# kehlert/ellp

Hardware: AMD Instinct MI355X
Metric: simplex pivots/sec (dense LP, primal, tableau resident in HBM) (higher is better)
Workload: dtype f64

## Files before the change

### ellp_amd/csrc/engine/ellp_engine.hip

```cpp
#include <hip/hip_runtime.h>
#include <dlfcn.h>
#include <rccl/rccl.h>

#include <algorithm>
#include <chrono>
#include <cmath>
#include <cstdarg>
#include <cstdint>
#include <cstdio>
#include <cstdlib>
#include <cstring>
#include <limits>
#include <memory>
#include <mutex>
#include <optional>
#include <vector>

#include "ellp_hip.h"
#include "ellp_lu_dev.h"

namespace {

constexpr int ST_RUNNING = 100;
constexpr int ST_NEED_MAINT = 101;
// ... 3064 lines not shown
void launch_dual_close(ellp_engine *e);
void maintain_inverse(ellp_engine *e, bool reactive = false, bool rebuild = false) {
    launch_dual_close(e);
    if (e->lagged) hipLaunchKernelGGL(k_drop_open, dim3(1), dim3(1), 0, e->stream, e->st);
    e->lag_open = false;
    if (rebuild) launch_refactor(e);
    else launch_refresh(e);
    const char *mode = getenv("ELLP_RESYNC");
    const bool want = mode && mode[0] == '0' ? false : (mode && mode[0] == '1' ? reactive : true);
    if (want) launch_resync(e, 0);
}

void reconcile_counters(ellp_engine *e) {
    const uint64_t ran = e->h_st->iters >= e->iters_seen ? e->h_st->iters - e->iters_seen : 0;
    const uint64_t lost = e->enqueued > ran ? e->enqueued - ran : 0;
    if (lost) {
        e->since_refactor = e->since_refactor > lost ? e->since_refactor - lost : 0;
        e->since_btran = e->since_btran > lost ? e->since_btran - lost : 0;
        e->since_drift = e->since_drift > lost ? e->since_drift - lost : 0;
    }
    e->enqueued = 0;
    e->iters_seen = e->h_st->iters;
}

void adopt_fin(ellp_engine *e) {
    if (e->h_st->status != ST_RUNNING || !e->h_st->fin) return;
    static int32_t fin_status;
    fin_status = e->h_st->fin - 1;
    (void)hipMemcpyAsync(&e->st->status, &fin_status, sizeof(int32_t), hipMemcpyHostToDevice, e->stream);
    (void)hipStreamSynchronize(e->stream);
    e->h_st->status = fin_status;
}

bool service_maintenance_request(ellp_engine *e) {
    if (e->h_st->status != ST_NEED_MAINT && !(e->h_st->status == ST_RUNNING && e->h_st->tiny)) return false;
    const int32_t running = ST_RUNNING, zero = 0;
    const bool rebuild = e->h_st->need_rebuild != 0;
    (void)hipMemcpyAsync(&e->st->status, &running, sizeof(int32_t), hipMemcpyHostToDevice, e->stream);
    (void)hipMemcpyAsync(&e->st->tiny, &zero, sizeof(int32_t), hipMemcpyHostToDevice, e->stream);
    (void)hipMemcpyAsync(&e->st->need_rebuild, &zero, sizeof(int32_t), hipMemcpyHostToDevice, e->stream);
    e->h_st->status = ST_RUNNING;
    e->h_st->tiny = 0;
    e->h_st->need_rebuild = 0;
    maintain_inverse(e, true, rebuild);
    e->maint_chain = 1;
    (void)hipStreamSynchronize(e->stream);
    e->maint_requests += 1;
    return true;
}

void launch_drift_check(ellp_engine *e) {
    if (e->drift_every <= 0) return;
    if (++e->since_drift < (uint64_t)e->drift_every) return;
    e->since_drift = 0;
    e->drift_checks += 1;
    DriftArgs a{e->A_B, e->A_N, e->d, e->colshard ? e->aq_cur : nullptr, e->upart, e->st, e->m, e->ld, e->btran_rows, e->btran_tiles, e->drift_tol};
    const int64_t half = e->ld >> 1;
    hipLaunchKernelGGL(k_drift_part, dim3((unsigned)((half + 255) / 256), (unsigned)e->btran_tiles), dim3(256), 0,
                       e->stream, a);
    hipLaunchKernelGGL(k_drift_reduce, dim3((unsigned)((e->m + WAVE - 1) / WAVE)), dim3(WAVE), 0, e->stream, a);
}

void launch_price2(ellp_engine *e, int use_pend) {
    Price2Args a{};
    a.p.A_N = e->A_N; a.p.W0 = e->W; a.p.W1 = e->W2; a.p.u = nullptr; a.p.c_N = e->c_N; a.p.Nb = e->Nb;
    a.p.N_index = e->N_index; a.p.dd = nullptr; a.p.xc = Xchg{e->X, e->seg, e->nbs, e->cpb}; a.p.st = e->st;
    a.p.ld = e->ld; a.p.nN = e->nN; a.p.cpb = e->cpb; a.p.block0 = e->rank * e->nbs; a.p.eps = e->eps;
    a.p.vs_row = e->vs_row; a.p.vs_val = e->vs_val; a.pos_hint = e->pos_hint;
    a.u0 = e->u; a.u1 = e->u + e->ld; a.W0 = e->W; a.W1 = e->W2;
    a.d = e->d; a.lam = e->lam; a.bmin = e->bmin; a.bsec = e->bmin + e->m; a.bidx = e->bidx; a.binfo = e->binfo; a.dpos = e->dpos;
    a.A_N = e->A_N; a.A_B = e->A_B; a.aq_save = e->aq_save; a.c_B = e->c_B; a.c_N = e->c_N; a.x = e->x;
    a.lb = e->lb; a.ub = e->ub; a.kind = e->kindv; a.B_index = e->B_index; a.N_index = e->N_index; a.Nb = e->Nb;
    a.m = e->m; a.rpb = e->upd2_rows; a.use_pend = use_pend; a.ill_tol = e->ill_tol;
    a.guard_abs = (e->cert_large && !e->guard_off) ? e->guard_abs : 0.0;
    a.aq_cur = e->colshard ? e->aq_cur : nullptr; a.own0 = e->own0; a.own1 = e->own1;
    a.trace = Trace{e->trace_obj, e->trace_it, e->trace_len};
    int mine = e->nblocks - a.p.block0;
    if (mine > e->nbs) mine = e->nbs;
    if (mine < 0) mine = 0;
    const dim3 g(mine + P2_BOOK), b(256);
    const size_t lds = e->price2_lds;
    if (e->colshard) {
        if (e->price_wave) {
            hipLaunchKernelGGL((k_price2_wave<true>), g, b, lds + sizeof(double) * (size_t)e->ld, e->stream, a);
            return;
        }
        if (e->price_nt) {
            switch (e->priceT) {
            case 1: hipLaunchKernelGGL((k_price2<1, true, true>), g, b, lds, e->stream, a); break;
            case 2: hipLaunchKernelGGL((k_price2<2, true, true>), g, b, lds, e->stream, a); break;
            case 4: hipLaunchKernelGGL((k_price2<4, true, true>), g, b, lds, e->stream, a); break;
            case 8: hipLaunchKernelGGL((k_price2<8, true, true>), g, b, lds, e->stream, a); break;
            default: hipLaunchKernelGGL((k_price2<16, true, true>), g, b, lds, e->stream, a); break;
            }
        } else {
            switch (e->priceT) {
            case 1: hipLaunchKernelGGL((k_price2<1, false, true>), g, b, lds, e->stream, a); break;
            case 2: hipLaunchKernelGGL((k_price2<2, false, true>), g, b, lds, e->stream, a); break;
            case 4: hipLaunchKernelGGL((k_price2<4, false, true>), g, b, lds, e->stream, a); break;
            case 8: hipLaunchKernelGGL((k_price2<8, false, true>), g, b, lds, e->stream, a); break;
            default: hipLaunchKernelGGL((k_price2<16, false, true>), g, b, lds, e->stream, a); break;
            }
        }
        return;
    }
    if (e->price_wave) {
        hipLaunchKernelGGL((k_price2_wave<false>), g, b, lds + sizeof(double) * (size_t)e->ld, e->stream, a);
        return;
    }
    if (e->price_nt) {
        switch (e->priceT) {
        case 1: hipLaunchKernelGGL((k_price2<1, true>), g, b, lds, e->stream, a); break;
        case 2: hipLaunchKernelGGL((k_price2<2, true>), g, b, lds, e->stream, a); break;
        case 4: hipLaunchKernelGGL((k_price2<4, true>), g, b, lds, e->stream, a); break;
        case 8: hipLaunchKernelGGL((k_price2<8, true>), g, b, lds, e->stream, a); break;
        default: hipLaunchKernelGGL((k_price2<16, true>), g, b, lds, e->stream, a); break;
        }
    } else {
        switch (e->priceT) {
        case 1: hipLaunchKernelGGL((k_price2<1, false>), g, b, lds, e->stream, a); break;
        case 2: hipLaunchKernelGGL((k_price2<2, false>), g, b, lds, e->stream, a); break;
        case 4: hipLaunchKernelGGL((k_price2<4, false>), g, b, lds, e->stream, a); break;
        case 8: hipLaunchKernelGGL((k_price2<8, false>), g, b, lds, e->stream, a); break;
        default: hipLaunchKernelGGL((k_price2<16, false>), g, b, lds, e->stream, a); break;
        }
    }
}

void launch_ftran_eta(ellp_engine *e) {
    FtranEtaArgs a{};
    a.W0 = e->W; a.W1 = e->W2; a.A_N = e->A_N; a.xc = Xchg{e->X, e->seg, e->nbs, e->cpb};
    a.N_index = e->N_index; a.B_index = e->B_index; a.Nb = e->Nb; a.kind = e->kindv;
    a.x = e->x; a.lb = e->lb; a.ub = e->ub; a.d = e->d; a.lam = e->lam; a.bmin = e->bmin; a.bsec = e->bmin + e->m; a.bidx = e->bidx;
    a.binfo = e->binfo; a.dpos = e->dpos;
    a.A_B = e->A_B; a.c_B = e->c_B; a.aq_save = e->aq_save; a.st = e->st; a.m = e->m; a.ld = e->ld; a.nN = e->nN;
    a.nblocks = e->nblocks; a.cpb = e->cpb; a.rows_per_block = e->upd2_rows; a.eps = e->eps;
    if (e->colshard) {
        a.aq_cur = e->aq_cur; a.aq_out = e->aq_cur;
        if (e->sel_in_ftran) {
            a.sel_packs = e->packs; a.sel_world = e->world; a.mbox_commit = e->sel_commit ? 1 : 0;
        }
    }
    const dim3 g(e->upd2_blocks + 1), b(256);
    const int64_t nr = ((e->ld >> 1) + 255) / 256;
    if (e->colshard) {
        if (nr <= 1) hipLaunchKernelGGL((k_ftran_eta<1, true>), g, b, e->ftran_lds, e->stream, a);
        else if (nr <= 2) hipLaunchKernelGGL((k_ftran_eta<2, true>), g, b, e->ftran_lds, e->stream, a);
        else if (nr <= 4) hipLaunchKernelGGL((k_ftran_eta<4, true>), g, b, e->ftran_lds, e->stream, a);
        else if (nr <= 8) hipLaunchKernelGGL((k_ftran_eta<8, true>), g, b, e->ftran_lds, e->stream, a);
        else hipLaunchKernelGGL((k_ftran_eta<0, true>), g, b, e->ftran_lds, e->stream, a);
        return;
    }
    const size_t hand_lds = ftran_col_offset(e->nblocks) + sizeof(double) * (size_t)e->ld;
    if (nr <= 1) hipLaunchKernelGGL((k_ftran_eta<1>), g, b, hand_lds, e->stream, a);
    else if (nr <= 2) hipLaunchKernelGGL((k_ftran_eta<2>), g, b, hand_lds, e->stream, a);
    else if (nr <= 4) hipLaunchKernelGGL((k_ftran_eta<4>), g, b, hand_lds, e->stream, a);
    else if (nr <= 8) hipLaunchKernelGGL((k_ftran_eta<8>), g, b, e->ftran_lds, e->stream, a);
    else hipLaunchKernelGGL((k_ftran_eta<0>), g, b, e->ftran_lds, e->stream, a);
}

void launch_primal_iteration_lagged(ellp_engine *e) {
    const bool full_btran = !e->u_valid || e->since_btran >= (uint64_t)e->btran_refresh;
    if (full_btran) {
        Prof p(e, ELLP_K_BTRAN);
        launch_btran(e);
        e->since_btran = 0;
        e->u_valid = true;
    }
    {
        Prof p(e, ELLP_K_PRICE);
        launch_price2(e, e->lag_open ? 1 : 0);
    }
    {
        Prof p(e, ELLP_K_FTRAN);
        launch_ftran_eta(e);
    }
    launch_drift_check(e);
    e->lag_open = true;
    e->since_btran += 1;
    e->since_refactor += 1;
    e->enqueued += 1;
}

void launch_dual_close(ellp_engine *e);
void launch_flush(ellp_engine *e) {
    launch_dual_close(e);
    if (!e->lag_open) return;
    {
        Prof p(e, ELLP_K_UPDATE);
        launch_update2<0>(e, 1);
    }
    e->lag_open = false;
}

void launch_price_se(ellp_engine *e) {
    SeArgs a{};
    a.A_N = e->A_N; a.u = e->u; a.rho = e->se_rho; a.v = e->se_v; a.c_N = e->c_N; a.Nb = e->Nb; a.N_index = e->N_index;
    a.gamma = e->se_gamma;
    const bool unit_ok = !(e->opts.flags & ELLP_FLAG_DENSE_PRICING);
    a.vs_row = unit_ok ? e->vs_row : nullptr; a.vs_val = unit_ok ? e->vs_val : nullptr;
    a.xc = Xchg{e->X, e->seg, e->nbs, e->cpb}; a.st = e->st; a.ld = e->ld; a.nN = e->nN; a.cpb = e->cpb; a.eps = e->eps;
    hipLaunchKernelGGL(k_price_se, dim3((unsigned)e->nblocks), dim3(256), 0, e->stream, a);
}

void launch_primal_iteration(ellp_engine *e) {
    if (e->lagged) {
        launch_primal_iteration_lagged(e);
        return;
    }
    const bool full_btran = (e->opts.btran_mode == 1) || !e->u_valid || e->since_btran >= (uint64_t)e->btran_refresh;
    if (full_btran) {
        Prof p(e, ELLP_K_BTRAN);
        launch_btran(e);
        e->since_btran = 0;
        e->u_valid = true;
    }
    {
        Prof p(e, ELLP_K_PRICE);
        if (e->se) launch_price_se(e);
        else launch_price<0>(e);
    }
    {
        Prof p(e, ELLP_K_FTRAN);
        launch_ftran2<0>(e);
    }
    if (e->se && !e->se_vpart) {
        Prof p(e, ELLP_K_BTRAN);
        launch_btran(e, e->d, e->se_v, e->se_v);
    }
    launch_drift_check(e);
    {
        Prof p(e, ELLP_K_UPDATE);
        launch_update2<0>(e, e->opts.btran_mode == 1 ? 0 : 1);
    }
    if (e->se && e->se_vpart) {
        Prof p(e, ELLP_K_BTRAN);
        hipLaunchKernelGGL(k_se_vreduce, dim3((unsigned)((e->ld + 15) / 16)), dim3(256), 0, e->stream, e->se_vpart, e->se_v, e->st, e->ld,
                           e->upd2_blocks);
    }
    e->since_btran += 1;
    e->since_refactor += 1;
    e->enqueued += 1;
}

void launch_dual_close(ellp_engine *e) {
    if (!e->dual_open) return;
    Prof p(e, ELLP_K_DUPDATE);
    DualCloseArgs c{e->d, e->A_N, e->A_B, e->c_B, e->c_N, e->x, e->dd, e->B_index, e->N_index, e->Nb, e->binfo, e->bmin,
                    e->bmin + e->m, (int)((e->m + UPD_ROWS - 1) / UPD_ROWS), e->st, e->m, e->ld, e->ill_tol,
                    Trace{e->trace_obj, e->trace_it, e->trace_len}, e->dual_maxviol};
    hipLaunchKernelGGL(k_dual_close, dim3(1), dim3(256), 0, e->stream, c);
    e->dual_open = false;
}

void launch_dual_fu(ellp_engine *e) {
    Prof p(e, ELLP_K_FTRAN);
    DualFuArgs a{};
    a.W0 = e->W; a.W1 = e->W2; a.A_N = e->A_N; a.xc = Xchg{e->X, e->seg, e->nbs, e->cpb};
    a.N_index = e->N_index; a.B_index = e->B_index; a.x = e->x; a.d = e->d; a.y = e->y; a.dd = e->dd;
    a.lb = e->lb; a.ub = e->ub; a.kind = e->kindv; a.lrow = e->binfo; a.ldelta = e->bmin; a.lside = e->bmin + e->m;
    a.st = e->st; a.m = e->m; a.ld = e->ld; a.nN = e->nN; a.nblocks = e->nblocks; a.eps = e->eps;
    a.seq = e->dual_seq;
    a.maxviol = e->dual_maxviol;
    a.guard_abs = (e->cert_large && !e->guard_off) ? e->guard_abs : 0.0;
    const dim3 g((unsigned)((e->m + UPD_ROWS - 1) / UPD_ROWS) + DFU_BOOK), b(256);
    const int64_t nr = ((e->ld >> 1) + 255) / 256;
    if (nr <= 1) hipLaunchKernelGGL((k_dual_fu<1>), g, b, 0, e->stream, a);
    else if (nr <= 2) hipLaunchKernelGGL((k_dual_fu<2>), g, b, 0, e->stream, a);
    else if (nr <= 4) hipLaunchKernelGGL((k_dual_fu<4>), g, b, 0, e->stream, a);
    else hipLaunchKernelGGL((k_dual_fu<8>), g, b, 0, e->stream, a);
    e->dual_open = true;
}

void launch_dual_iteration(ellp_engine *e) {
    e->dual_seq += 1;
    {
        Prof p(e, ELLP_K_DPRICE);
        launch_price<1>(e);
    }
    const bool drift_now = e->drift_every > 0 && e->since_drift + 1 >= (uint64_t)e->drift_every;
    if (e->dual_fused && !drift_now) {
        if (e->drift_every > 0) e->since_drift += 1;
        launch_dual_fu(e);
        if (!e->dual_fold) launch_dual_close(e);
        e->since_refactor += 1;
        e->enqueued += 1;
        return;
    }
    {
        Prof p(e, ELLP_K_FTRAN);
        launch_ftran2<1>(e);
    }
    launch_drift_check(e);
    {
        Prof p(e, ELLP_K_DUPDATE);
        launch_update2<1>(e, 0);
    }
    e->since_refactor += 1;
    e->enqueued += 1;
}

void launch_dleave(ellp_engine *e) {
    Prof p(e, ELLP_K_DLEAVE);
    DLeaveArgs a{e->x, e->lb, e->ub, e->kindv, e->B_index, e->st, e->m, e->eps, e->dual_maxviol};
    hipLaunchKernelGGL(k_dleave, dim3(1), dim3(256), 0, e->stream, a);
}

ellp_status status_message(const DevState &s, char *errbuf, size_t errlen) {
    switch (s.status) {
// ... 2636 lines not shown
```

### ellp_amd/csrc/engine/ellp_lagged.inc

```

struct Price2Args {
    PriceArgs p;
    double *u0, *u1;
    double *W0, *W1;
    const double *d, *lam, *bmin, *bsec;
    const int32_t *bidx, *binfo;
    const uint8_t *dpos;
    double *A_N, *A_B, *aq_save, *c_B, *c_N, *x;
    const double *lb, *ub;
    const uint8_t *kind;
    int64_t *B_index, *N_index;
    uint8_t *Nb;
    int64_t m;
    int rpb;
    int use_pend;
    uint8_t *pos_hint;
    const double *aq_cur;
    int64_t own0, own1;
    double ill_tol;
    double guard_abs;
    Trace trace;
};

struct PHead {
// ... 904 lines not shown

    if (row_block) {
        double acc0[2 * UPD_ROWS], acc1[2 * UPD_ROWS];
#pragma unroll
        for (int k = 0; k < 2 * UPD_ROWS; ++k) acc0[k] = acc1[k] = 0.0;
        if (NR > 0) {
            double2 cq[NRR];
            if (!EARLY) {
                const double2 *rho2 = reinterpret_cast<const double2 *>(src + (apply ? r : 0) * a.ld);
#pragma unroll
                for (int u = 0; u < NR; ++u) {
                    const int64_t t = tid + 256 * u;
                    const int64_t tc = t < half ? t : 0;
                    const double2 pv = rho2[tc];
                    const double2 cv = col[tc];
                    pr[u] = (apply && t < half) ? pv : make_double2(0.0, 0.0);
                    cq[u] = (have_col && t < half) ? cv : make_double2(0.0, 0.0);
                }
            }
            if (apply) {
#pragma unroll
                for (int k = 0; k < UPD_ROWS; ++k) {
                    const int64_t i = row0 + k;
                    if (!(k < R && i < m)) continue;
                    const double f = (i != r) ? -(dv[k] / d_r) : 0.0;
                    double2 *drow = reinterpret_cast<double2 *>(dst + i * a.ld);
#pragma unroll
                    for (int u = 0; u < NR; ++u) {
                        const int64_t t = tid + 256 * u;
                        if (t >= half) continue;
                        double2 o;
                        if (i == r) {
                            o = make_double2(pr[u].x / alpha_r, pr[u].y / alpha_r);
                        } else {
                            o.x = fma(f, pr[u].x, wreg[k][u].x);
                            o.y = fma(f, pr[u].y, wreg[k][u].y);
                        }
                        store_row2<true>(drow + t, o);
                        wreg[k][u] = o;
                    }
                }
            }
            STAMP(1, 2);
            if (EARLY) {
#pragma unroll
                for (int u = 0; u < NR; ++u) {
                    const int64_t t = tid + 256 * u;
                    const double2 cv = col[t < half ? t : 0];
                    cq[u] = (have_col && t < half) ? cv : make_double2(0.0, 0.0);
                }
            }
#pragma unroll
            for (int k = 0; k < UPD_ROWS; ++k) {
                const int64_t i = row0 + k;
                if (!(k < R && i < m)) continue;
#pragma unroll
                for (int u = 0; u < NR; ++u) {
                    acc0[k] = fma(wreg[k][u].x, cq[u].x, acc0[k]);
                    acc1[k] = fma(wreg[k][u].y, cq[u].y, acc1[k]);
                }
            }
        } else {
            eta_ftran_rows_stream(src, dst, col, have_col, m, a.ld, apply != 0, r, dv, d_r, alpha_r, row0, R < UPD_ROWS ? R : UPD_ROWS,
                                  tid, acc0, acc1);
        }
        if (R > UPD_ROWS)
            eta_ftran_rows_stream(src, dst, col, have_col, m, a.ld, apply != 0, r, dv2, d_r, alpha_r, row0 + UPD_ROWS, R - UPD_ROWS, tid,
                                  acc0 + UPD_ROWS, acc1 + UPD_ROWS);
        if (have_col) {
#pragma unroll
            for (int k = 0; k < 2 * UPD_ROWS; ++k) {
                const double s = wave_sum(acc0[k] + acc1[k]);
                if (lane == 0) s_dot[wave][k] = s;
            }
            __syncthreads();
            STAMP(1, 3);
            double li = INFINITY;
            if (own) {
                const int k = tid;
                const double di = sgn * (((s_dot[0][k] + s_dot[1][k]) + s_dot[2][k]) + s_dot[3][k]);
                const double xi = xi0, lbi = lbi0, ubi = ubi0;
                a.d[myrow] = di;
                li = primal_lambda(di, xi, lbi, ubi, k0, a.eps);
                if (li != li) st->nan_flag = 1;
                a.lam[myrow] = li;
                a.bidx[myrow] = (int32_t)bi0;
                a.dpos[myrow] = di > 0.0 ? 1 : 0;
            }
            if (tid < 2 * UPD_ROWS) {
                s_lam[tid] = li;
                s_dp[tid] = own ? (a.dpos[myrow] ? 1 : 0) : 0;
            }
            __syncthreads();
            if (tid == 0) {
                double m1 = INFINITY, m2 = INFINITY;
                int info = -1;
                for (int k = 0; k < R; ++k) {
                    const double v = s_lam[k];
                    if (v < m1) {
                        m2 = m1;
                        m1 = v;
                        info = (int)(2 * (row0 + k)) + s_dp[k];
                    } else if (v < m2) {
                        m2 = v;
                    }
                }
                a.bmin[blockIdx.x - NBK] = m1;
                a.bsec[blockIdx.x - NBK] = m2;
                a.binfo[blockIdx.x - NBK] = info;
            }
            STAMP(1, 4);
        }
        return;
    }
    if (SH && sel_rec) {
        double2 *dstc = reinterpret_cast<double2 *>(a.aq_out);
        for (int64_t t = tid; t < half; t += 256) dstc[t] = col[t];
    }
    if (st->mv_pending) {
        const int64_t mr = st->mv_r;
        double2 *cb = reinterpret_cast<double2 *>(a.A_B + mr * a.ld);
        const double2 *sv = reinterpret_cast<const double2 *>(a.aq_save);
        for (int64_t t = tid; t < half; t += 256) cb[t] = sv[t];
        if (tid == 0) a.c_B[mr] = st->cq_save;
    }
    if (tid == 0) {
        const int new_cur = apply ? (src_sel ^ 1) : src_sel;
        if (st->tiny_p) {
            st->tiny_p = 0;
            st->tiny = 1;
        }
        st->mv_pending = 0;
        st->cur = new_cur;
        st->usel = st->usel_next;
        st->s_cur = new_cur;
        st->iters += 1;
        st->open = q < 0 ? 0 : 1;
        if (q < 0) {
            st->fin = ELLP_OPTIMAL + 1;
        } else {
            const int64_t jq = a.N_index[q];
            ELLP_CHECK(st, q < a.nN, 9111);
            st->s_q = q;
            st->s_at_lower = at_lower;
            st->s_nbq = a.Nb[q];
            st->s_jq = jq;
            st->s_rq = sel_rec ? sel_rec[3] : (aq_in ? st->sh_rq : a.xc.r(q));
            const int kk = a.kind[jq];
            st->s_lambda0 = (kk == ELLP_BOUND_TWOSIDED) ? a.ub[jq] - a.lb[jq] : (kk == ELLP_BOUND_FIXED ? 0.0 : INFINITY);
        }
    }
}


__device__ __forceinline__ void wave_lds_sync() { asm volatile("s_waitcnt lgkmcnt(0)" ::: "memory"); }
template <class T>
__device__ __forceinline__ void retire_here(T &v) { asm volatile("" : "+v"(v)); }
__host__ __device__ constexpr size_t ftran_col_offset(int nblocks) { return (sizeof(double) * (size_t)nblocks + 16 + 15) & ~(size_t)15; }

template <int K>
__device__ __forceinline__ void wave_sum_rows(double s[UPD_ROWS]) {
#pragma unroll
    for (int o = 32; o > 0; o >>= 1) {
        double t[K];
#pragma unroll
        for (int k = 0; k < K; ++k) t[k] = __shfl_xor(s[k], o);
#pragma unroll
        for (int k = 0; k < K; ++k) s[k] += t[k];
    }
}

template <int NR>
__device__ __forceinline__ void ftran_eta_handoff(const FtranEtaArgs &a) {
    static_assert(NR >= 1 && NR <= 4, "rows of at most 2,048 doubles: at most UPD_ROWS rows per block");
    extern __shared__ __align__(16) unsigned char smem[];
    __shared__ long long s_q;
    __shared__ int s_leave, s_atl, s_nh, s_band;
    __shared__ int s_hblk[FC_SLOTS];
    __shared__ double s_hkey[FC_SLOTS * 64];
    __shared__ int32_t s_hidx[FC_SLOTS * 64];
    __shared__ double s_dot[4][UPD_ROWS];
    __shared__ double s_lam[UPD_ROWS];
    __shared__ int s_dp[UPD_ROWS];
    DevState *st = a.st;
    STAMP(1, 0);
    const int tid = threadIdx.x, lane = tid & 63;
    const int wave = __builtin_amdgcn_readfirstlane(tid >> 6);
    if (tid == 0) s_leave = st->status != ST_RUNNING ? 1 : (st->nan_flag ? 2 : 0);
    const int src_sel = st->f_src;
    const int apply = st->pe_valid;
    const int64_t r = st->pe_r;
    const double d_r = st->pe_d_r, alpha_r = st->pe_alpha_r;
    const double *src = src_sel ? a.W1 : a.W0;
    double *dst = src_sel ? a.W0 : a.W1;
    const int64_t half = a.ld >> 1, m = a.m;
    constexpr int NBK = 1;
    const bool row_block = blockIdx.x >= NBK;
    const int R = a.rows_per_block;
    const int64_t row0 = ((int64_t)blockIdx.x - NBK) * R;
    double *s_bk = reinterpret_cast<double *>(smem);
    double2 *s_col = reinterpret_cast<double2 *>(smem + ftran_col_offset(a.nblocks));

    constexpr int FB = 16;
    double v0[FB];
    const int64_t myrow = row0 + tid;
    const bool own = row_block && tid < R && myrow < m;
    int64_t bi0 = 0;
    if (wave == 0) {
        const double *pb[FB];
#pragma unroll
        for (int u = 0; u < FB; ++u) {
            const int b = lane + 64 * u;
            pb[u] = &a.xc.bk(b < a.nblocks ? b : 0);
        }
        __builtin_amdgcn_sched_barrier(0);
#pragma unroll
        for (int u = 0; u < FB; ++u) v0[u] = *pb[u];
        bi0 = a.B_index[own ? myrow : 0];
    }
    __builtin_amdgcn_sched_barrier(0);
    double dv[UPD_ROWS];
#pragma unroll
    for (int k = 0; k < UPD_ROWS; ++k) dv[k] = (row_block && k < R && row0 + k < m) ? a.d[row0 + k] : 0.0;
    double2 wreg[UPD_ROWS][NR], pr[NR];
#pragma unroll
    for (int k = 0; k < UPD_ROWS; ++k) {
        const int64_t i = row0 + k;
        const bool ok = row_block && k < R && i < m;
        const double2 *srow = reinterpret_cast<const double2 *>(src + (ok ? i : 0) * a.ld);
#pragma unroll
        for (int u = 0; u < NR; ++u) {
            const int64_t t = tid + 256 * u;
            wreg[k][u] = srow[t < half ? t : 0];
        }
    }
    {
        const double2 *rho2 = reinterpret_cast<const double2 *>(src + (apply ? r : 0) * a.ld);
#pragma unroll
        for (int u = 0; u < NR; ++u) {
            const int64_t t = tid + 256 * u;
            pr[u] = rho2[t < half ? t : 0];
        }
    }
    double xi0 = 0.0, lbi0 = 0.0, ubi0 = 0.0;
    int k0 = 0;
    lds_barrier();
    const int leave = s_leave;
    if (leave) {
        if (leave == 2 && blockIdx.x == 0 && tid == 0) st->status = ELLP_ERR_NAN;
        return;
    }

    auto eta_store = [&]() {
        if (!apply) return;
#pragma unroll
        for (int k = 0; k < UPD_ROWS; ++k) {
            const int64_t i = row0 + k;
            if (!(k < R && i < m)) continue;
            const double f = (i != r) ? -(dv[k] / d_r) : 0.0;
            double2 *drow = reinterpret_cast<double2 *>(dst + i * a.ld);
#pragma unroll
            for (int u = 0; u < NR; ++u) {
                const int64_t t = tid + 256 * u;
                if (t >= half) continue;
                double2 o;
                if (i == r) {
                    o = make_double2(pr[u].x / alpha_r, pr[u].y / alpha_r);
                } else {
                    o.x = fma(f, pr[u].x, wreg[k][u].x);
                    o.y = fma(f, pr[u].y, wreg[k][u].y);
                }
                store_row2<true>(drow + t, o);
                wreg[k][u] = o;
            }
        }
    };

    auto rows_retired = [&]() {
#pragma unroll
        for (int k = 0; k < UPD_ROWS; ++k) {
            retire_here(dv[k]);
#pragma unroll
            for (int u = 0; u < NR; ++u) {
                retire_here(wreg[k][u].x);
                retire_here(wreg[k][u].y);
            }
        }
#pragma unroll
        for (int u = 0; u < NR; ++u) {
            retire_here(pr[u].x);
            retire_here(pr[u].y);
        }
        __builtin_amdgcn_s_waitcnt(0x0F70);
    };

    if (wave == 0) {
        xi0 = a.x[bi0];
        lbi0 = a.lb[bi0];
        ubi0 = a.ub[bi0];
        k0 = a.kind[bi0];
        double tmax = -INFINITY;
#pragma unroll
        for (int u = 0; u < FB; ++u) {
            const bool in = lane + 64 * u < a.nblocks;
            if (in) s_bk[lane + 64 * u] = v0[u];
            tmax = fmax(tmax, in ? v0[u] : -INFINITY);
        }
        for (int b0 = lane + 64 * FB; b0 < a.nblocks; b0 += 64 * FB) {
            double v[FB];
#pragma unroll
            for (int u = 0; u < FB; ++u) {
                const int b = b0 + 64 * u;
                const double t = a.xc.bk(b < a.nblocks ? b : 0);
                v[u] = b < a.nblocks ? t : -INFINITY;
            }
#pragma unroll
            for (int u = 0; u < FB; ++u) {
                if (b0 + 64 * u < a.nblocks) s_bk[b0 + 64 * u] = v[u];
                tmax = fmax(tmax, v[u]);
            }
        }
        if (lane == 0) {
            s_nh = 0;
            s_band = 0;
        }
        const double M = wave_allmax_dpp(tmax);
        wave_lds_sync();
        STAMP(1, 5);
        for (int b = lane; b < a.nblocks; b += 64) {
            const double v = s_bk[b];
            if (M - v < 4.0 * a.eps) {
                const int slot = atomicAdd(&s_nh, 1);
                if (slot < FC_SLOTS) s_hblk[slot] = b;
            } else if (M - v < 6.0 * a.eps) {
                s_band = 1;
            }
        }
        wave_lds_sync();
        STAMP(1, 6);
        const int nh = s_nh;
        const bool fast = M > -INFINITY && nh <= FC_SLOTS && !s_band;
        if (fast) {
            if (lane == 0) {
                for (int i = 1; i < nh; ++i) {
                    const int v = s_hblk[i];
                    int j = i - 1;
                    while (j >= 0 && s_hblk[j] > v) {
                        s_hblk[j + 1] = s_hblk[j];
                        --j;
                    }
                    s_hblk[j + 1] = v;
                }
            }
            wave_lds_sync();
            for (int sl = 0; sl < nh; ++sl) {
                const int64_t j = (int64_t)s_hblk[sl] * a.cpb + lane;
                const bool ok = lane < a.cpb && j < a.nN;
                const int64_t jc = ok ? j : 0;
                const double kl = a.xc.key(jc);
                const int64_t il = a.N_index[jc];
                const double kv = ok ? kl : -INFINITY;
                s_hkey[sl * 64 + lane] = kv;
                s_hidx[sl * 64 + lane] = ok ? (int32_t)il : 0;
                if (M - kv < 6.0 * a.eps && !(M - kv < 4.0 * a.eps)) s_band = 1;
            }
            wave_lds_sync();
        }
        long long q = -1;
        bool done = false;
        if (fast && !s_band) {
            FoldState f{false, 0.0, 0, -1};
            for (int sl = 0; sl < nh; ++sl)
                fold_elements(f, s_hkey[sl * 64 + lane], s_hidx[sl * 64 + lane], (int64_t)s_hblk[sl] * a.cpb, a.eps, lane);
            q = f.qacc;
            done = true;
        }
        if (!done && M > -INFINITY) q = entering_fold_full(s_bk, a.nblocks, a.cpb, a.nN, a.xc, a.N_index, a.eps, lane);
        STAMP(1, 1);
        const bool hc = q >= 0;
        int nbq = a.Nb[hc ? q : 0];
        if (row_block && hc) {
            const double2 *col = reinterpret_cast<const double2 *>(a.A_N + q * a.ld);
            double2 cv[4 * NR];
#pragma unroll
            for (int u = 0; u < 4 * NR; ++u) {
                const int64_t t = lane + 64 * u;
                cv[u] = col[t < half ? t : 0];
            }
            __builtin_amdgcn_sched_barrier(0);
#pragma unroll
            for (int u = 0; u < 4 * NR; ++u) {
                retire_here(cv[u].x);
                retire_here(cv[u].y);
            }
#pragma unroll
            for (int u = 0; u < 4 * NR; ++u) {
                const int64_t t = lane + 64 * u;
                if (t < half) s_col[t] = cv[u];
            }
        }
        retire_here(nbq);
        retire_here(xi0);
        retire_here(lbi0);
        retire_here(ubi0);
        retire_here(k0);
        if (lane == 0) {
            s_q = q;
            s_atl = hc ? (nbq == ELLP_NB_LOWER ? 1 : 0) : 0;
        }
        STAMP(1, 7);
    }
    rows_retired();
    if (wave != 0 && row_block) {
        eta_store();
        STAMP_AT(1, 2, 64);
    }
    lds_barrier();
    const long long q = s_q;
    const bool have_col = q >= 0;
    const int at_lower = s_atl;

    if (!row_block) {
        if (st->mv_pending) {
            const int64_t mr = st->mv_r;
            double2 *cb = reinterpret_cast<double2 *>(a.A_B + mr * a.ld);
            const double2 *sv = reinterpret_cast<const double2 *>(a.aq_save);
            for (int64_t t = tid; t < half; t += 256) cb[t] = sv[t];
            if (tid == 0) a.c_B[mr] = st->cq_save;
        }
        if (tid == 0) {
            const int new_cur = apply ? (src_sel ^ 1) : src_sel;
            if (st->tiny_p) {
                st->tiny_p = 0;
                st->tiny = 1;
            }
            st->mv_pending = 0;
            st->cur = new_cur;
            st->usel = st->usel_next;
            st->s_cur = new_cur;
            st->iters += 1;
            st->open = q < 0 ? 0 : 1;
            if (q < 0) {
                st->fin = ELLP_OPTIMAL + 1;
            } else {
                const int64_t jq = a.N_index[q];
                ELLP_CHECK(st, q < a.nN, 9111);
                st->s_q = q;
                st->s_at_lower = at_lower;
                st->s_nbq = a.Nb[q];
                st->s_jq = jq;
                st->s_rq = a.xc.r(q);
                const int kk = a.kind[jq];
                st->s_lambda0 = (kk == ELLP_BOUND_TWOSIDED) ? a.ub[jq] - a.lb[jq] : (kk == ELLP_BOUND_FIXED ? 0.0 : INFINITY);
            }
        }
        return;
    }
    if (wave == 0) eta_store();
    if (!have_col) return;

    double acc0[UPD_ROWS], acc1[UPD_ROWS];
#pragma unroll
    for (int k = 0; k < UPD_ROWS; ++k) acc0[k] = acc1[k] = 0.0;
    double2 cq[NR];
#pragma unroll
    for (int u = 0; u < NR; ++u) {
        const int64_t t = tid + 256 * u;
        const double2 cv = s_col[t < half ? t : 0];
        cq[u] = t < half ? cv : make_double2(0.0, 0.0);
    }
#pragma unroll
    for (int k = 0; k < UPD_ROWS; ++k) {
        const int64_t i = row0 + k;
        if (!(k < R && i < m)) continue;
#pragma unroll
        for (int u = 0; u < NR; ++u) {
            const bool in = tid + 256 * u < half;
            acc0[k] = fma(in ? wreg[k][u].x : 0.0, cq[u].x, acc0[k]);
            acc1[k] = fma(in ? wreg[k][u].y : 0.0, cq[u].y, acc1[k]);
        }
    }
    double s[UPD_ROWS];
#pragma unroll
    for (int k = 0; k < UPD_ROWS; ++k) s[k] = acc0[k] + acc1[k];
    if (R >= 3) wave_sum_rows<4>(s);
    else if (R == 2) wave_sum_rows<2>(s);
    else wave_sum_rows<1>(s);
    if (lane == 0) {
#pragma unroll
        for (int k = 0; k < UPD_ROWS; ++k) s_dot[wave][k] = s[k];
    }
    lds_barrier();
    STAMP(1, 3);
    if (wave != 0) return;
    const double sgn = at_lower ? -1.0 : 1.0;
    double li = INFINITY;
    int dp = 0;
    if (own) {
        const int k = tid;
        const double di = sgn * (((s_dot[0][k] + s_dot[1][k]) + s_dot[2][k]) + s_dot[3][k]);
        a.d[myrow] = di;
        li = primal_lambda(di, xi0, lbi0, ubi0, k0, a.eps);
        if (li != li) st->nan_flag = 1;
        dp = di > 0.0 ? 1 : 0;
        a.lam[myrow] = li;
        a.bidx[myrow] = (int32_t)bi0;
        a.dpos[myrow] = (uint8_t)dp;
    }
    if (tid < UPD_ROWS) {
        s_lam[tid] = li;
        s_dp[tid] = dp;
    }
    wave_lds_sync();
    if (tid == 0) {
        double m1 = INFINITY, m2 = INFINITY;
        int info = -1;
        for (int k = 0; k < R; ++k) {
            const double v = s_lam[k];
            if (v < m1) {
                m2 = m1;
                m1 = v;
                info = (int)(2 * (row0 + k)) + s_dp[k];
            } else if (v < m2) {
                m2 = v;
            }
        }
        a.bmin[blockIdx.x - NBK] = m1;
        a.bsec[blockIdx.x - NBK] = m2;
        a.binfo[blockIdx.x - NBK] = info;
    }
    STAMP(1, 4);
}

constexpr bool ftran_eta_hands_off(int NR, bool SH) { return !SH && NR >= 1 && NR <= 4; }

template <int NR, bool SH = false>
__global__ __launch_bounds__(256) void k_ftran_eta(FtranEtaArgs a) {
    if constexpr (ftran_eta_hands_off(NR, SH)) ftran_eta_handoff<NR>(a);
    else ftran_eta_whole<NR, SH>(a);
}
```

Before: 27890.

## Dedicate wave 0 to pivot selection and add a fifth wave for row work

The handoff FTRAN/eta kernel now launches 320 threads instead of 256. Wave 0 only does the control path: block-key loads, pivot selection and the final lambda/min reduction. Four extra waves (indexed by sid = tid-64) load rows, do the eta store, the dot-product accumulation and the pending column move. This lets wave 0's serial selection overlap with the row loads and eta stores the other waves used to share with it, at the cost of more threads per block, extra barriers and more complex synchronisation between waves.

New measurement: 28740 (median of 6 runs). 1.03x the previous value.

```diff
diff --git a/ellp_amd/csrc/engine/ellp_engine.hip b/ellp_amd/csrc/engine/ellp_engine.hip
--- a/ellp_amd/csrc/engine/ellp_engine.hip
+++ b/ellp_amd/csrc/engine/ellp_engine.hip
@@ -3240,9 +3240,13 @@
         return;
     }
     const size_t hand_lds = ftran_col_offset(e->nblocks) + sizeof(double) * (size_t)e->ld;
-    if (nr <= 1) hipLaunchKernelGGL((k_ftran_eta<1>), g, b, hand_lds, e->stream, a);
-    else if (nr <= 2) hipLaunchKernelGGL((k_ftran_eta<2>), g, b, hand_lds, e->stream, a);
-    else if (nr <= 4) hipLaunchKernelGGL((k_ftran_eta<4>), g, b, hand_lds, e->stream, a);
+    const dim3 bh(FTRAN_HAND_THREADS);
+    static_assert(ftran_eta_threads(1, false) == FTRAN_HAND_THREADS && ftran_eta_threads(4, false) == FTRAN_HAND_THREADS &&
+                      ftran_eta_threads(8, false) == 256 && ftran_eta_threads(4, true) == 256,
+                  "320 threads exactly where hand_lds is used");
+    if (nr <= 1) hipLaunchKernelGGL((k_ftran_eta<1>), g, bh, hand_lds, e->stream, a);
+    else if (nr <= 2) hipLaunchKernelGGL((k_ftran_eta<2>), g, bh, hand_lds, e->stream, a);
+    else if (nr <= 4) hipLaunchKernelGGL((k_ftran_eta<4>), g, bh, hand_lds, e->stream, a);
     else if (nr <= 8) hipLaunchKernelGGL((k_ftran_eta<8>), g, b, e->ftran_lds, e->stream, a);
     else hipLaunchKernelGGL((k_ftran_eta<0>), g, b, e->ftran_lds, e->stream, a);
 }
diff --git a/ellp_amd/csrc/engine/ellp_lagged.inc b/ellp_amd/csrc/engine/ellp_lagged.inc
--- a/ellp_amd/csrc/engine/ellp_lagged.inc
+++ b/ellp_amd/csrc/engine/ellp_lagged.inc
@@ -1080,6 +1080,7 @@
     }
 }
 
+constexpr int FTRAN_HAND_THREADS = 320;
 
 __device__ __forceinline__ void wave_lds_sync() { asm volatile("s_waitcnt lgkmcnt(0)" ::: "memory"); }
 template <class T>
@@ -1114,6 +1115,7 @@
     STAMP(1, 0);
     const int tid = threadIdx.x, lane = tid & 63;
     const int wave = __builtin_amdgcn_readfirstlane(tid >> 6);
+    const int sid = tid - 64;
     if (tid == 0) s_leave = st->status != ST_RUNNING ? 1 : (st->nan_flag ? 2 : 0);
     const int src_sel = st->f_src;
     const int apply = st->pe_valid;
@@ -1134,50 +1136,10 @@
     const int64_t myrow = row0 + tid;
     const bool own = row_block && tid < R && myrow < m;
     int64_t bi0 = 0;
-    if (wave == 0) {
-        const double *pb[FB];
-#pragma unroll
-        for (int u = 0; u < FB; ++u) {
-            const int b = lane + 64 * u;
-            pb[u] = &a.xc.bk(b < a.nblocks ? b : 0);
-        }
-        __builtin_amdgcn_sched_barrier(0);
-#pragma unroll
-        for (int u = 0; u < FB; ++u) v0[u] = *pb[u];
-        bi0 = a.B_index[own ? myrow : 0];
-    }
-    __builtin_amdgcn_sched_barrier(0);
-    double dv[UPD_ROWS];
-#pragma unroll
-    for (int k = 0; k < UPD_ROWS; ++k) dv[k] = (row_block && k < R && row0 + k < m) ? a.d[row0 + k] : 0.0;
-    double2 wreg[UPD_ROWS][NR], pr[NR];
-#pragma unroll
-    for (int k = 0; k < UPD_ROWS; ++k) {
-        const int64_t i = row0 + k;
-        const bool ok = row_block && k < R && i < m;
-        const double2 *srow = reinterpret_cast<const double2 *>(src + (ok ? i : 0) * a.ld);
-#pragma unroll
-        for (int u = 0; u < NR; ++u) {
-            const int64_t t = tid + 256 * u;
-            wreg[k][u] = srow[t < half ? t : 0];
-        }
-    }
-    {
-        const double2 *rho2 = reinterpret_cast<const double2 *>(src + (apply ? r : 0) * a.ld);
-#pragma unroll
-        for (int u = 0; u < NR; ++u) {
-            const int64_t t = tid + 256 * u;
-            pr[u] = rho2[t < half ? t : 0];
-        }
-    }
     double xi0 = 0.0, lbi0 = 0.0, ubi0 = 0.0;
     int k0 = 0;
-    lds_barrier();
-    const int leave = s_leave;
-    if (leave) {
-        if (leave == 2 && blockIdx.x == 0 && tid == 0) st->status = ELLP_ERR_NAN;
-        return;
-    }
+    double dv[UPD_ROWS];
+    double2 wreg[UPD_ROWS][NR], pr[NR];
 
     auto eta_store = [&]() {
         if (!apply) return;
@@ -1189,7 +1151,7 @@
             double2 *drow = reinterpret_cast<double2 *>(dst + i * a.ld);
 #pragma unroll
             for (int u = 0; u < NR; ++u) {
-                const int64_t t = tid + 256 * u;
+                const int64_t t = sid + 256 * u;
                 if (t >= half) continue;
                 double2 o;
                 if (i == r) {
@@ -1222,7 +1184,32 @@
         __builtin_amdgcn_s_waitcnt(0x0F70);
     };
 
+    auto block0_move = [&]() {
+        if (!st->mv_pending) return;
+        const int64_t mr = st->mv_r;
+        double2 *cb = reinterpret_cast<double2 *>(a.A_B + mr * a.ld);
+        const double2 *sv = reinterpret_cast<const double2 *>(a.aq_save);
+        for (int64_t t = tid; t < half; t += FTRAN_HAND_THREADS) cb[t] = sv[t];
+        if (tid == 0) a.c_B[mr] = st->cq_save;
+    };
+
     if (wave == 0) {
+        const double *pb[FB];
+#pragma unroll
+        for (int u = 0; u < FB; ++u) {
+            const int b = lane + 64 * u;
+            pb[u] = &a.xc.bk(b < a.nblocks ? b : 0);
+        }
+        __builtin_amdgcn_sched_barrier(0);
+#pragma unroll
+        for (int u = 0; u < FB; ++u) v0[u] = *pb[u];
+        bi0 = a.B_index[own ? myrow : 0];
+        lds_barrier();
+        const int leave = s_leave;
+        if (leave) {
+            if (leave == 2 && blockIdx.x == 0 && tid == 0) st->status = ELLP_ERR_NAN;
+            return;
+        }
         xi0 = a.x[bi0];
         lbi0 = a.lb[bi0];
         ubi0 = a.ub[bi0];
@@ -1337,11 +1324,74 @@
             s_atl = hc ? (nbq == ELLP_NB_LOWER ? 1 : 0) : 0;
         }
         STAMP(1, 7);
-    }
-    rows_retired();
-    if (wave != 0 && row_block) {
-        eta_store();
-        STAMP_AT(1, 2, 64);
+    } else {
+#pragma unroll
+        for (int k = 0; k < UPD_ROWS; ++k) dv[k] = (row_block && k < R && row0 + k < m) ? a.d[row0 + k] : 0.0;
+#pragma unroll
+        for (int k = 0; k < UPD_ROWS; ++k) {
+            const int64_t i = row0 + k;
+            const bool ok = row_block && k < R && i < m;
+            const double2 *srow = reinterpret_cast<const double2 *>(src + (ok ? i : 0) * a.ld);
+#pragma unroll
+            for (int u = 0; u < NR; ++u) {
+                const int64_t t = sid + 256 * u;
+                wreg[k][u] = srow[t < half ? t : 0];
+            }
+        }
+        {
+            const double2 *rho2 = reinterpret_cast<const double2 *>(src + (apply ? r : 0) * a.ld);
+#pragma unroll
+            for (int u = 0; u < NR; ++u) {
+                const int64_t t = sid + 256 * u;
+                pr[u] = rho2[t < half ? t : 0];
+            }
+        }
+        lds_barrier();
+        if (s_leave) return;
+        rows_retired();
+        if (row_block) {
+            eta_store();
+            STAMP_AT(1, 2, 64);
+        }
+        lds_barrier();
+        if (!row_block) {
+            block0_move();
+            return;
+        }
+        if (s_q < 0) return;
+        double acc0[UPD_ROWS], acc1[UPD_ROWS];
+#pragma unroll
+        for (int k = 0; k < UPD_ROWS; ++k) acc0[k] = acc1[k] = 0.0;
+        double2 cq[NR];
+#pragma unroll
+        for (int u = 0; u < NR; ++u) {
+            const int64_t t = sid + 256 * u;
+            const double2 cv = s_col[t < half ? t : 0];
+            cq[u] = t < half ? cv : make_double2(0.0, 0.0);
+        }
+#pragma unroll
+        for (int k = 0; k < UPD_ROWS; ++k) {
+            const int64_t i = row0 + k;
+            if (!(k < R && i < m)) continue;
+#pragma unroll
+            for (int u = 0; u < NR; ++u) {
+                const bool in = sid + 256 * u < half;
+                acc0[k] = fma(in ? wreg[k][u].x : 0.0, cq[u].x, acc0[k]);
+                acc1[k] = fma(in ? wreg[k][u].y : 0.0, cq[u].y, acc1[k]);
+            }
+        }
+        double s[UPD_ROWS];
+#pragma unroll
+        for (int k = 0; k < UPD_ROWS; ++k) s[k] = acc0[k] + acc1[k];
+        if (R >= 3) wave_sum_rows<4>(s);
+        else if (R == 2) wave_sum_rows<2>(s);
+        else wave_sum_rows<1>(s);
+        if (lane == 0) {
+#pragma unroll
+            for (int k = 0; k < UPD_ROWS; ++k) s_dot[wave - 1][k] = s[k];
+        }
+        lds_barrier();
+        return;
     }
     lds_barrier();
     const long long q = s_q;
@@ -1349,13 +1399,7 @@
     const int at_lower = s_atl;
 
     if (!row_block) {
-        if (st->mv_pending) {
-            const int64_t mr = st->mv_r;
-            double2 *cb = reinterpret_cast<double2 *>(a.A_B + mr * a.ld);
-            const double2 *sv = reinterpret_cast<const double2 *>(a.aq_save);
-            for (int64_t t = tid; t < half; t += 256) cb[t] = sv[t];
-            if (tid == 0) a.c_B[mr] = st->cq_save;
-        }
+        block0_move();
         if (tid == 0) {
             const int new_cur = apply ? (src_sel ^ 1) : src_sel;
             if (st->tiny_p) {
@@ -1384,43 +1428,9 @@
         }
         return;
     }
-    if (wave == 0) eta_store();
     if (!have_col) return;
-
-    double acc0[UPD_ROWS], acc1[UPD_ROWS];
-#pragma unroll
-    for (int k = 0; k < UPD_ROWS; ++k) acc0[k] = acc1[k] = 0.0;
-    double2 cq[NR];
-#pragma unroll
-    for (int u = 0; u < NR; ++u) {
-        const int64_t t = tid + 256 * u;
-        const double2 cv = s_col[t < half ? t : 0];
-        cq[u] = t < half ? cv : make_double2(0.0, 0.0);
-    }
-#pragma unroll
-    for (int k = 0; k < UPD_ROWS; ++k) {
-        const int64_t i = row0 + k;
-        if (!(k < R && i < m)) continue;
-#pragma unroll
-        for (int u = 0; u < NR; ++u) {
-            const bool in = tid + 256 * u < half;
-            acc0[k] = fma(in ? wreg[k][u].x : 0.0, cq[u].x, acc0[k]);
-            acc1[k] = fma(in ? wreg[k][u].y : 0.0, cq[u].y, acc1[k]);
-        }
-    }
-    double s[UPD_ROWS];
-#pragma unroll
-    for (int k = 0; k < UPD_ROWS; ++k) s[k] = acc0[k] + acc1[k];
-    if (R >= 3) wave_sum_rows<4>(s);
-    else if (R == 2) wave_sum_rows<2>(s);
-    else wave_sum_rows<1>(s);
-    if (lane == 0) {
-#pragma unroll
-        for (int k = 0; k < UPD_ROWS; ++k) s_dot[wave][k] = s[k];
-    }
     lds_barrier();
     STAMP(1, 3);
-    if (wave != 0) return;
     const double sgn = at_lower ? -1.0 : 1.0;
     double li = INFINITY;
     int dp = 0;
@@ -1461,9 +1471,10 @@
 }
 
 constexpr bool ftran_eta_hands_off(int NR, bool SH) { return !SH && NR >= 1 && NR <= 4; }
+constexpr int ftran_eta_threads(int NR, bool SH) { return ftran_eta_hands_off(NR, SH) ? FTRAN_HAND_THREADS : 256; }
 
 template <int NR, bool SH = false>
-__global__ __launch_bounds__(256) void k_ftran_eta(FtranEtaArgs a) {
+__global__ __launch_bounds__(ftran_eta_threads(NR, SH)) void k_ftran_eta(FtranEtaArgs a) {
     if constexpr (ftran_eta_hands_off(NR, SH)) ftran_eta_handoff<NR>(a);
     else ftran_eta_whole<NR, SH>(a);
 }
```
